# Priberam/Enhance-CB-Whisper

Hardware: AMD Instinct MI355X
Metric: utterances/sec (30 s clips) + keywords/sec matched, Whisper-large-v3 LEF 10k kw (higher is better)
Workload: dtype bf16

## Files before the change

enhance-cb-whisper_amd/cbw/_lib.py:

```python
from __future__ import annotations

import ctypes
import os

import torch

_HERE = os.path.dirname(os.path.abspath(__file__))
LIB_PATH = os.environ.get("CBW_LIB", os.path.join(_HERE, "libcbw.so"))

c_int, c_int64, c_float, c_void_p, c_char_p = ctypes.c_int, ctypes.c_int64, ctypes.c_float, ctypes.c_void_p, ctypes.c_char_p


class KwsConfig(ctypes.Structure):
    _fields_ = [("n_layers", c_int), ("embedding_dim", c_int), ("variant", c_int), ("proj_units", c_int),
                ("resnet_depth", c_int)]


class EncoderConfig(ctypes.Structure):
    _fields_ = [("n_mel", c_int), ("d_model", c_int), ("n_layers", c_int), ("n_heads", c_int), ("ffn_dim", c_int)]


class DecoderConfig(ctypes.Structure):
    _fields_ = [("vocab", c_int), ("d_model", c_int), ("n_layers", c_int), ("n_heads", c_int), ("ffn_dim", c_int),
                ("max_len", c_int)]
# ... 73 lines not shown
    "cbw_decoder_prefill": (c_int, [c_void_p, c_void_p, c_int, c_int, c_int, c_void_p, c_int64, c_void_p, c_void_p]),
    "cbw_decoder_cross_kv_slot": (c_int, [c_void_p, c_void_p, c_int, c_int, c_void_p, c_int64, c_int, c_void_p]),
    "cbw_decoder_prefill_rows": (c_int, [c_void_p, c_void_p, c_int, c_int, c_int, c_int, c_int, c_int, c_void_p, c_int64,
                                         c_void_p, c_void_p]),
    "cbw_decoder_step_rows": (c_int, [c_void_p, c_void_p, c_void_p, c_int, c_int, c_void_p, c_int64, c_void_p, c_void_p]),
    "cbw_decoder_reorder": (c_int, [c_void_p, c_void_p, c_int, c_int, c_int, c_void_p, c_int64, c_void_p]),
    "cbw_decoder_cross_attn_probs": (c_int, [c_void_p, c_void_p, c_int, c_void_p, c_int, c_int, c_int, c_void_p,
                                             c_int64, c_void_p, c_void_p]),
    "cbw_dtw": (c_int, [c_void_p, c_int, c_int, c_void_p, c_void_p, c_void_p]),
    "cbw_logprob_topk": (c_int, [c_void_p, c_int, c_int, c_int, c_void_p, c_int64, c_int, c_void_p, c_void_p, c_void_p]),
    "cbw_timestamp_rules": (c_int, [c_void_p, c_int, c_int, c_int, c_void_p, c_void_p, c_int, c_int, c_int, c_int,
                                    c_void_p, c_void_p]),
    "cbw_kws_profile_read": (c_int, [c_void_p, ctypes.POINTER(ctypes.c_double), ctypes.POINTER(ctypes.c_double), ctypes.POINTER(c_int)]),
    "cbw_kws_profile_records": (c_int, [c_void_p, c_void_p, c_void_p, c_void_p, c_int]),
    "cbw_kws_profile_tiers": (c_int, [c_void_p, c_void_p, c_int]),
    "cbw_kws_profile_kernels": (c_int, [c_void_p, c_void_p, c_int]),
    "cbw_kws_calibrate_fp8": (c_int, [c_void_p, c_void_p, c_void_p, c_void_p, c_void_p, c_int, c_int, c_int, c_void_p,
                                      c_int, c_float, c_void_p, c_int64, c_void_p]),
    "cbw_kws_score_fp8": (c_int, [c_void_p, c_void_p, c_void_p, c_void_p, c_void_p, c_int, c_int, c_int, c_void_p,
                                  c_int, c_void_p, c_int64, c_void_p]),
    "cbw_kws_set_score_offset_fp8": (c_int, [c_void_p, c_void_p]),
    "cbw_kws_fp8_scales": (c_int, [c_void_p, c_void_p, c_int]),
    "cbw_conv2d_fp8": (c_int, [c_void_p] * 5 + [c_float, c_void_p, c_float] + [c_int] * 9 + [c_void_p]),
    "cbw_fp8_probe": (c_int, [c_int, c_void_p, c_void_p, c_void_p, c_void_p, c_int, c_void_p]),
    "cbw_conv2d_f32": (c_int, [c_void_p] * 5 + [c_int] * 12 + [c_void_p]),
    "cbw_sim_maps_f32": (c_int, [c_void_p, c_void_p, c_int, c_void_p, c_void_p] + [c_int] * 5 + [c_void_p, c_void_p, c_int,
                                 c_void_p, c_int, c_int, c_void_p, c_void_p]),
    "cbw_maxpool_f32": (c_int, [c_void_p, c_void_p, c_int, c_int, c_int, c_int, c_void_p]),
    "cbw_pool_fc_f32": (c_int, [c_void_p] * 4 + [c_int, c_int, c_void_p, c_int, c_int, c_void_p]),
    "cbw_split3_f32": (c_int, [c_void_p, c_void_p, c_int64, c_int, c_void_p]),
    "cbw_channel_sum_workspace_bytes": (c_int64, [c_int]),
    "cbw_channel_sum_f32": (c_int, [c_void_p, c_int64, c_int, c_void_p, c_int64, c_void_p]),
    "cbw_conv2d_x3": (c_int, [c_void_p] * 4 + [c_int, c_void_p, c_void_p] + [c_int] * 9 + [c_void_p]),
}

ERRORS = {-1: "CBW_ERR_INVALID", -2: "CBW_ERR_HIP", -3: "CBW_ERR_OOM", -4: "CBW_ERR_STATE", -5: "CBW_ERR_NOT_FOUND"}

_lib = None


class CbwError(RuntimeError):
    pass


def load() -> ctypes.CDLL:
    global _lib
    if _lib is None:
        if not os.path.exists(LIB_PATH):
            raise CbwError(f"libcbw.so not found at {LIB_PATH}; build it with `python -c 'import __graft_entry__ as g; "
                           f"g.build()'` (hipcc --offload-arch=gfx950)")
        lib = ctypes.CDLL(LIB_PATH)
        for name, (res, args) in SIGNATURES.items():
            fn = getattr(lib, name)
            fn.restype = res
            fn.argtypes = args
        _lib = lib
    return _lib


def check(rc: int, what: str) -> None:
    if rc != 0:
        msg = load().cbw_last_error()
        msg = msg.decode() if msg else ""
        err = ValueError if rc == -1 else CbwError
        raise err(f"{what} failed with {ERRORS.get(rc, rc)}: {msg}")

# ... 25 lines not shown
```

enhance-cb-whisper_amd/csrc/cbw_kernels.h:

```cpp
#pragma once
#include <hip/hip_runtime.h>
#include <stdint.h>

#include <initializer_list>
#include <string>

typedef __bf16 bf16;

enum {
    CBW_EPI_RELU = 1,
    CBW_EPI_GELU = 2,
    CBW_EPI_RES_F32 = 4,
    CBW_EPI_OUT_F32 = 8,
    CBW_EPI_RES_AFTER_ACT = 16,
    CBW_EPI_SPLIT3 = 32,
    CBW_EPI_RES_SPLIT = 64
};

struct ConvArgs {
    const void* x;
    const void* w;
    const float* bias;
    const void* res;
    void* y;
    const void* zero;
    int N, H, W, Cin, Ho, Wo, Cout, KH, KW;
    int sh, sw, ph, pw;
    int M;
    int res_ld, y_ld;
    int flags;
    const void* x2;
    int Cin2, H2, W2, s2;
    int ksplit;
    float* partial;
    float* y32;
    int x_ld, xfold;
};

hipError_t cbw_conv_igemm(const ConvArgs& a, hipStream_t st);
extern thread_local const char* cbw_last_conv_kernel;
extern thread_local int cbw_cs_grid_cus;
inline std::string kernel_name(const char* base, std::initializer_list<int> targs) {
    std::string s = std::string(base) + "<";
    bool first = true;
    for (int t : targs) {
        s += (first ? "" : ", ") + std::to_string(t);
        first = false;
    }
    return s + ">";
}
int cbw_conv_splitk_factor(const ConvArgs& a);
hipError_t cbw_conv_igemm_splitk(const ConvArgs& a, int ksplit, float* partial, hipStream_t st);
struct GemvArgs {
    const bf16* x;
    int ldx;
    const bf16* w;
    const float* bias;
    const void* res;
    int res_ld;
    void* y;
    int ldy;
    int M, N, K, flags;
    const float* xf;
    const float* ln_g;
    const float* ln_b;
    float ln_eps;
    bf16* kv_k;
    bf16* kv_v;
    int64_t kv_ld;
// ... 148 lines not shown
```

enhance-cb-whisper_amd/csrc/conv_igemm.hip:

```cpp
#include "cbw_common.h"
#include "cbw_kernels.h"

thread_local const char* cbw_last_conv_kernel = "";

namespace {

constexpr int BK = 64;
constexpr int EPI_LD = 68;
constexpr int EPI_BYTES = 4 * 64 * EPI_LD * 4;
template <int BM, int BN>
constexpr int lds_bytes() { return 2 * (BM + BN) * 128 > EPI_BYTES ? 2 * (BM + BN) * 128 : EPI_BYTES; }

CBW_DEV int swz(int r) { return (r >> 1) & 7; }

CBW_DEV void store_out8(const ConvArgs& a, int flags, int m, int col, const float (&v)[8]) {
    if (flags & CBW_EPI_SPLIT3) {
        bf16x8 hi, lo;
#pragma unroll
        for (int q = 0; q < 8; ++q) {
            hi[q] = f2bf(v[q]);
            lo[q] = f2bf(v[q] - bf2f(hi[q]));
        }
        bf16* yp = (bf16*)a.y + (int64_t)m * a.y_ld + col;
        *(bf16x8*)yp = hi;
// ... 232 lines not shown
#pragma unroll
            for (int q = 0; q < 8; ++q) v[q] = fmaxf(v[q], 0.f);
        } else if (flags & CBW_EPI_GELU) {
#pragma unroll
            for (int q = 0; q < 8; ++q) v[q] = gelu_erf(v[q]);
        }
        if (has_res && (flags & CBW_EPI_RES_AFTER_ACT))
#pragma unroll
            for (int q = 0; q < 8; ++q) v[q] += rv[q];
        store_out8(a, flags, m, col, v);
    }
}

template <int BM, int BN, int KH, int KW>
__global__ __launch_bounds__(256, 2) void conv_igemm_persist(ConvArgs a, int ntiles) {
    static_assert((BM / 64) * (BN / 64) == 4, "4 waves x 64x64 tiles");
    static_assert(KH * KW <= 32, "tap mask");
    constexpr int STAGE = (BM + BN) * 128;
    constexpr int WN = BN / 64;
    constexpr int AR = BM / 32;
    constexpr int BR = BN / 32;
    extern __shared__ __attribute__((aligned(16))) char smem[];

    const int tid = threadIdx.x, lane = tid & 63, wid = tid >> 6;
    const int wm = wid / WN, wn = wid % WN;
    float* E = (float*)(smem + 2 * STAGE) + wid * 8 * EPI_LD;
    const int nt_n = a.Cout / BN;
    const int cin2 = (KH * KW == 1 && a.x2 != nullptr) ? a.Cin2 : 0;
    const int Ktot = KH * KW * a.Cin + cin2;
    const int csteps = a.Cin / BK;
    const int nsteps = KH * KW * csteps + cin2 / BK;
    const int HoWo = a.Ho * a.Wo;
    const int xld = a.x_ld ? a.x_ld : a.Cin;
    const int G = gridDim.x;
    const int my_tiles = (ntiles - (int)blockIdx.x + G - 1) / G;
    const int total = my_tiles * nsteps;
    const int sub_r = lane >> 3, chunk = lane & 7;
    auto tile_of = [&](int ti) { return xcd_remap(ti * G + (int)blockIdx.x, ntiles); };

    int64_t a_base[AR];
    int64_t a_base2[(KH * KW == 1) ? AR : 1];
    int a_ih0[AR], a_iw0[AR];
    bool a_ok[AR];
    const bf16* wrow[BR];
    const bool dual = (KH * KW == 1) && a.x2 != nullptr;
    const int csteps1 = csteps;
    auto setup_issue_tile = [&](int ti) {
        const int tile = tile_of(ti);
        const int m0 = (tile / nt_n) * BM, n0 = (tile % nt_n) * BN;
#pragma unroll
        for (int j = 0; j < AR; ++j) {
            const int r = (wid * AR + j) * 8 + sub_r;
            const int m = m0 + r;
            a_ok[j] = m < a.M;
            const int mm = a_ok[j] ? m : 0;
            const int n = mm / HoWo, rem = mm - n * HoWo;
            const int oh = rem / a.Wo, ow = rem - oh * a.Wo;
            a_ih0[j] = oh * a.sh - a.ph;
            a_iw0[j] = ow * a.sw - a.pw;
            a_base[j] = (int64_t)n * a.H * a.W * xld;
            if constexpr (KH * KW == 1)
                if (dual) a_base2[j] = (((int64_t)n * a.H2 + oh * a.s2) * a.W2 + ow * a.s2) * a.Cin2;
        }
#pragma unroll
        for (int j = 0; j < BR; ++j) {
            const int r = (wid * BR + j) * 8 + sub_r;
            wrow[j] = (const bf16*)a.w + (int64_t)(n0 + r) * Ktot + ((chunk ^ swz(r)) * 8);
        }
    };
    auto issue_stage = [&](int s, int buf) {
        const int tap = s / csteps;
        const int c0 = fold_c((s - tap * csteps) * BK, a.xfold);
        const int kh = tap / KW, kw = tap - kh * KW;
        char* A = smem + buf * STAGE;
        char* B = A + BM * 128;
        const bool second = dual && s >= csteps1;
#pragma unroll
        for (int j = 0; j < AR; ++j) {
            const int rb = wid * AR + j;
            const int r = rb * 8 + sub_r;
            const void* src;
            const int ih = a_ih0[j] + kh, iw = a_iw0[j] + kw;
            bool ok = a_ok[j];
            if constexpr (KH * KW > 1) ok = ok && ih >= 0 && ih < a.H && iw >= 0 && iw < a.W;
            if (!ok)
                src = a.zero;
            else if constexpr (KH * KW == 1) {
                if (second)
                    src = (const bf16*)a.x2 + a_base2[j] + (s - csteps1) * BK + ((chunk ^ swz(r)) * 8);
                else
                    src = (const bf16*)a.x + a_base[j] + ((int64_t)ih * a.W + iw) * xld + c0 + ((chunk ^ swz(r)) * 8);
            } else
                src = (const bf16*)a.x + a_base[j] + ((int64_t)ih * a.W + iw) * xld + c0 + ((chunk ^ swz(r)) * 8);
            __builtin_amdgcn_global_load_lds(src, (void*)(A + rb * 1024), 16, 0, 0);
        }
#pragma unroll
        for (int j = 0; j < BR; ++j) {
            const int rb = wid * BR + j;
            __builtin_amdgcn_global_load_lds((const void*)(wrow[j] + (int64_t)s * BK), (void*)(B + rb * 1024), 16, 0, 0);
        }
    };

    const int ecg = lane & 7, erow = lane >> 3;
    const bool res_bf16 = a.res != nullptr && !(a.flags & (CBW_EPI_RES_F32 | CBW_EPI_RES_SPLIT));
    bf16x8 rpre[8];
    f32x4 bias0, bias1;
    auto prefetch_epi = [&](int tile) {
        const int m0 = (tile / nt_n) * BM, n0 = (tile % nt_n) * BN;
        const int ecol = n0 + wn * 64 + ecg * 8;
#pragma unroll
        for (int it = 0; it < 8; ++it) {
            const int m = m0 + wm * 64 + it * 8 + erow;
            if (res_bf16 && m < a.M)
                rpre[it] = *(const bf16x8*)((const bf16*)a.res + (int64_t)m * a.res_ld + ecol);
            else
                rpre[it] = bf16x8{};
        }
        bias0 = f32x4{0.f, 0.f, 0.f, 0.f};
        bias1 = f32x4{0.f, 0.f, 0.f, 0.f};
        if (a.bias) {
            bias0 = *(const f32x4*)(a.bias + ecol);
            bias1 = *(const f32x4*)(a.bias + ecol + 4);
// ... 298 lines not shown
CBW_DEV int p8_off(int r, int c) { return r * 128 + ((c ^ ((r >> 1) & 7)) << 4); }
template <int BN> struct P8Shape {
    static constexpr int BM = 65536 / BN;
    static constexpr int NA = BM / 128, NB = BN / 128;
    static constexpr int WCN = BN / 64;
    static constexpr int BUF = (BM + BN) * 128;
};
template <int N> CBW_DEV void vm_wait() {
    static_assert(N >= 0 && N <= 15, "vm_wait");
    asm volatile("s_waitcnt vmcnt(%0)" ::"n"(N) : "memory");
}

template <int KH, int KW, int BN = 256>
__global__ __launch_bounds__(512, 1) void conv_igemm_p8(ConvArgs a) {
    static_assert(KH * KW <= 32, "tap mask");
    using S = P8Shape<BN>;
    constexpr int BM = S::BM, NA = S::NA, NB = S::NB, WCN = S::WCN;
    extern __shared__ __attribute__((aligned(16))) char smem[];
    const int tid = threadIdx.x, lane = tid & 63, wid = tid >> 6;
    const int wr = (wid >> 2) * (4 / WCN) + (wid & 3) / WCN, wc = (wid & 3) % WCN;
    const int fr = lane & 15, fq = lane >> 4;
    const int nt_n = a.Cout / BN;
    const int nt_m = (a.M + BM - 1) / BM;
    const int bid = xcd_remap(blockIdx.x, nt_m * nt_n);
    const int tm = bid / nt_n, tn = bid % nt_n;
    const int m0 = tm * BM, n0 = tn * BN;
    const int cin2 = a.x2 ? a.Cin2 : 0;
    const int Ktot = KH * KW * a.Cin + cin2;
    const int csteps = a.Cin / P8_BK;
    const int nk1 = KH * KW * csteps;
    const int nk = nk1 + cin2 / P8_BK;
    const int HoWo = a.Ho * a.Wo;
    const int xld = a.x_ld ? a.x_ld : a.Cin;

    const int sub = lane >> 3, pch = lane & 7;
    const bf16* a_px[2][NA];
    const bf16* a2_px[2][NA];
    unsigned a_tm[2][NA];
    const bf16* wrow[2][NB];
#pragma unroll
    for (int h = 0; h < 2; ++h)
#pragma unroll
        for (int g = 0; g < NA; ++g) {
            const int r = g * 128 + h * 64 + wid * 8 + sub;
            const int m = m0 + r;
            const bool okm = m < a.M;
            const int mm = okm ? m : 0;
            const int n = mm / HoWo, rem = mm - n * HoWo;
            const int oh = rem / a.Wo, ow = rem - oh * a.Wo;
            const int ih0 = oh * a.sh - a.ph, iw0 = ow * a.sw - a.pw;
            a2_px[h][g] = a.x2 ? (const bf16*)a.x2 + (((int64_t)n * a.H2 + oh * a.s2) * a.W2 + ow * a.s2) * cin2 +
                                     ((pch ^ ((r >> 1) & 7)) * 8)
                               : nullptr;
            unsigned tmask = 0;
#pragma unroll
            for (int kh = 0; kh < KH; ++kh)
#pragma unroll
                for (int kw = 0; kw < KW; ++kw) {
                    const int ih = ih0 + kh, iw = iw0 + kw;
                    if (okm && ih >= 0 && ih < a.H && iw >= 0 && iw < a.W) tmask |= 1u << (kh * KW + kw);
                }
            a_tm[h][g] = tmask;
            a_px[h][g] = (const bf16*)a.x + (int64_t)n * a.H * a.W * xld + ((int64_t)ih0 * a.W + iw0) * xld +
                         ((pch ^ ((r >> 1) & 7)) * 8);
        }
#pragma unroll
    for (int h = 0; h < 2; ++h)
#pragma unroll
        for (int g = 0; g < NB; ++g) {
            const int rb = h * (BN / 2) + g * 64 + wid * 8 + sub;
            const int rs = (rb & ~31) | (((rb & 15) >> 2) << 3) | (((rb >> 4) & 1) << 2) | (rb & 3);
            wrow[h][g] = (const bf16*)a.w + (int64_t)(n0 + rs) * Ktot + ((pch ^ ((rb >> 1) & 7)) * 8);
        }
    int nx_cs = 0, nx_tap = 0, nx_kh = 0, nx_kw = 0;
    int nx_off = fold_c(0, a.xfold);
    auto advance = [&]() {
        if (++nx_cs == csteps) {
            nx_cs = 0;
            ++nx_tap;
            if (++nx_kw == KW) { nx_kw = 0; ++nx_kh; }
        }
        nx_off = (nx_kh * a.W + nx_kw) * xld + fold_c(nx_cs * P8_BK, a.xfold);
    };
    auto issue = [&](int kt, int which) {
        char* A = smem + (kt & 1) * S::BUF;
        if (which == 0 || which == 3) {
            const int h = which == 3;
            if (kt >= nk1) {
                const int c0 = (kt - nk1) * P8_BK;
#pragma unroll
                for (int g = 0; g < NA; ++g) {
                    const void* src = (a_tm[h][g] & 1u) ? (const void*)(a2_px[h][g] + c0) : a.zero;
                    __builtin_amdgcn_global_load_lds(src, (void*)(A + (g * 128 + h * 64 + wid * 8) * 128), 16, 0, 0);
                }
                return;
            }
            const int tap = nx_tap;
            const int toff = nx_off;
#pragma unroll
            for (int g = 0; g < NA; ++g) {
                const void* src = ((a_tm[h][g] >> tap) & 1u) ? (const void*)(a_px[h][g] + toff) : a.zero;
                __builtin_amdgcn_global_load_lds(src, (void*)(A + (g * 128 + h * 64 + wid * 8) * 128), 16, 0, 0);
            }
        } else {
            const int h = which - 1;
            char* B = A + BM * 128;
#pragma unroll
            for (int g = 0; g < NB; ++g)
                __builtin_amdgcn_global_load_lds((const void*)(wrow[h][g] + (int64_t)kt * P8_BK),
                                                 (void*)(B + (h * (BN / 2) + g * 64 + wid * 8) * 128), 16, 0, 0);
        }
    };

    f32x4 acc[8][4];
#pragma unroll
    for (int i = 0; i < 8; ++i)
#pragma unroll
        for (int j = 0; j < 4; ++j) acc[i][j] = f32x4{0.f, 0.f, 0.f, 0.f};
    bf16x8 av[4][2], bv[2][2];

#pragma unroll
    for (int w = 0; w < 4; ++w) issue(0, w);
// ... 162 lines not shown

template <int BM, int BN, int KH, int KW>
hipError_t launch_persist(const ConvArgs& a, hipStream_t st) {
    const int ntiles = ((a.M + BM - 1) / BM) * (a.Cout / BN);
    int G = 2 * num_cus();
    if (ntiles < G) G = ntiles;
    constexpr int lds = 2 * (BM + BN) * 128 + 4 * 8 * EPI_LD * 4;
    static const std::string nm = kernel_name("conv_igemm_persist", {BM, BN, KH, KW});
    cbw_last_conv_kernel = nm.c_str();
    hipLaunchKernelGGL((conv_igemm_persist<BM, BN, KH, KW>), dim3(G), dim3(256), lds, st, a, ntiles);
    return hipGetLastError();
}

template <int BM, int BN, int KH, int KW>
hipError_t launch_t(const ConvArgs& a, hipStream_t st) {
    const int nt = ((a.M + BM - 1) / BM) * (a.Cout / BN);
    constexpr int lds = lds_bytes<BM, BN>();
    static const std::string nm = kernel_name("conv_igemm_kernel", {BM, BN, KH, KW});
    cbw_last_conv_kernel = nm.c_str();
    hipLaunchKernelGGL((conv_igemm_kernel<BM, BN, KH, KW>), dim3(nt), dim3(256), lds, st, a);
    return hipGetLastError();
}

bool ring_wanted(const ConvArgs& a) {
    if (!cbw_conv_ring_supported(a)) return false;
    const int ktot = a.KH * a.KW * a.Cin + (a.x2 ? a.Cin2 : 0);
    return a.KH * a.KW == 1 && a.res == nullptr && ktot <= 768;
}

template <int KH, int KW>
hipError_t launch_k(const ConvArgs& a, hipStream_t st) {
    const int64_t xld = a.x_ld ? a.x_ld : a.Cin;
    if (((int64_t)(KH - 1) * a.W + (KW - 1)) * xld + a.Cin + (a.x2 ? a.Cin2 : 0) > INT32_MAX) return hipErrorInvalidValue;
    const bool tile_only = a.xfold || (a.x_ld && a.x_ld != a.Cin) || (a.flags & (CBW_EPI_SPLIT3 | CBW_EPI_RES_SPLIT));
    const bool p8_fit = p8_mode() == 1 && a.res == nullptr && a.Cout % P8_BN == 0 && a.Cin % P8_BK == 0 &&
                        a.xfold % P8_BK == 0 && KH * KW * a.Cin + (a.x2 ? a.Cin2 : 0) >= 512 &&
                        (a.x2 == nullptr || (KH * KW == 1 && a.Cin2 % P8_BK == 0 && !a.xfold && !a.x_ld)) &&
                        !(a.flags & (CBW_EPI_OUT_F32 | CBW_EPI_GELU | CBW_EPI_RES_SPLIT)) &&
                        ((a.M + P8_BM - 1) / P8_BM) * (a.Cout / P8_BN) >= num_cus();
    const int px2 = p8_x2();
    if (p8_fit && a.x2 && px2 >= 2) return launch_p8<KH, KW>(a, st);
    if (!tile_only && KH * KW == 1 && cbw_conv_stream_wanted(a)) return cbw_conv_stream(a, st);
    if (p8_fit && a.x2 && px2 >= 1) return launch_p8<KH, KW>(a, st);
    if (p8_tier_enabled() && (a.flags & (CBW_EPI_SPLIT3 | CBW_EPI_OUT_F32)) && a.xfold && a.x2 == nullptr &&
        p8_mode() == 1 && a.Cout % P8_BN == 0 && a.Cin % P8_BK == 0 && a.xfold % P8_BK == 0 &&
        !(a.flags & (CBW_EPI_GELU | CBW_EPI_RES_AFTER_ACT))) {
        const int ktot = KH * KW * a.Cin;
        const int tiles = ((a.M + P8_BM - 1) / P8_BM) * (a.Cout / P8_BN);
        if (ktot >= 512 && (tiles >= num_cus() || (ktot >= 4096 && 2 * tiles >= num_cus())))
            return launch_p8<KH, KW>(a, st);
    }
    if (!tile_only && ring_wanted(a)) return cbw_conv_ring(a, st);
    const bool big_ok = a.res == nullptr && a.x2 == nullptr &&
                        !(a.flags & (CBW_EPI_OUT_F32 | CBW_EPI_GELU | CBW_EPI_RES_SPLIT)) &&
                        a.Cin % BIG_BK == 0 && a.xfold % BIG_BK == 0 && KH * KW * a.Cin >= 256;
    const int big_tiles = ((a.M + BIG_BM - 1) / BIG_BM) * (a.Cout / 256);
    if (big_ok && big_tiles >= num_cus()) {
        if (a.Cout % 256 == 0 && p8_mode() == 1 && a.Cin % P8_BK == 0 && a.xfold % P8_BK == 0)
            return launch_p8<KH, KW>(a, st);
        if (a.Cout % 256 == 0) return launch_big<256, KH, KW>(a, st);
    }
    if (big_ok && p8_n128() && p8_mode() == 1 && a.Cout % 256 == 128 && a.Cin % P8_BK == 0 && a.xfold % P8_BK == 0 &&
        KH * KW * a.Cin >= 512 && ((a.M + 511) / 512) * (a.Cout / 128) >= num_cus())
        return launch_p8<KH, KW, 128>(a, st);
    if (a.Cout % 128 == 0) {
        const bool short_k = a.KH * a.KW * (a.Cin / BK) == 1;
        if (a.x2 != nullptr || short_k || a.res != nullptr)
            return launch_persist<128, 128, KH, KW>(a, st);
        return launch_t<128, 128, KH, KW>(a, st);
    }
    if (a.x2 != nullptr) return hipErrorInvalidValue;
    return launch_t<256, 64, KH, KW>(a, st);
}

}

namespace {
__global__ __launch_bounds__(256) void splitk_epilogue_kernel(ConvArgs a, int S) {
    const int64_t n4 = (int64_t)a.M * a.Cout / 4;
    for (int64_t e = blockIdx.x * (int64_t)blockDim.x + threadIdx.x; e < n4; e += (int64_t)gridDim.x * blockDim.x) {
        const int64_t i = e * 4;
        const int m = (int)(i / a.Cout), col = (int)(i - (int64_t)m * a.Cout);
// ... 33 lines not shown
    }
}
}

int cbw_conv_splitk_factor(const ConvArgs& a) {
    if (a.KH != 1 || a.KW != 1 || a.x2 != nullptr || a.Cout % 128 || a.Cin % BK) return 1;
    const int tiles = ((a.M + 127) / 128) * (a.Cout / 128);
    const int slots = 2 * num_cus();
    const int nsteps = a.Cin / BK;
    int S = 1;
    while (S < 8 && tiles * (S * 2) <= slots && nsteps / (S * 2) >= 4) S *= 2;
    return S;
}

hipError_t cbw_conv_igemm_splitk(const ConvArgs& a0, int ksplit, float* partial, hipStream_t st) {
    if (ksplit <= 1 || partial == nullptr) return cbw_conv_igemm(a0, st);
    if (a0.KH != 1 || a0.KW != 1 || a0.x2 != nullptr || a0.Cout % 128 || a0.Cin % BK || a0.Cout % 4 ||
        a0.y_ld % 4 || (a0.res && a0.res_ld % 4) || ksplit > a0.Cin / BK)
        return hipErrorInvalidValue;
    ConvArgs a = a0;
    a.ksplit = ksplit;
    a.partial = partial;
    const int nt = ((a.M + 127) / 128) * (a.Cout / 128);
    constexpr int lds = lds_bytes<128, 128>();
    cbw_last_conv_kernel = "conv_igemm_kernel<128, 128, 1, 1> + splitk_epilogue_kernel";
    hipLaunchKernelGGL((conv_igemm_kernel<128, 128, 1, 1>), dim3(nt, ksplit), dim3(256), lds, st, a);
    const int64_t n4 = (int64_t)a.M * a.Cout / 4;
    const int grid = (int)std::min<int64_t>((n4 + 255) / 256, 4 * num_cus());
    hipLaunchKernelGGL(splitk_epilogue_kernel, dim3(grid), dim3(256), 0, st, a, ksplit);
    return hipGetLastError();
}

hipError_t cbw_conv_igemm(const ConvArgs& a, hipStream_t st) {
    if (a.x2 != nullptr && (a.KH != 1 || a.KW != 1 || a.Cin2 % BK)) return hipErrorInvalidValue;
    if (a.KH == 1 && a.KW == 1) return launch_k<1, 1>(a, st);
    if (a.KH == 3 && a.KW == 3) return launch_k<3, 3>(a, st);
    if (a.KH == 1 && a.KW == 3) return launch_k<1, 3>(a, st);
    return hipErrorInvalidValue;
}
```

enhance-cb-whisper_amd/csrc/runtime.cpp:

```cpp
#include <hip/hip_runtime.h>

#include <algorithm>
#include <cmath>
#include <cstring>
#include <limits>
#include <map>
#include <memory>
#include <string>
#include <vector>

#include "cbw.h"
#include "cbw_kernels.h"

namespace {

thread_local std::string g_err;

int fail(int code, const std::string& msg) {
    g_err = msg;
    return code;
}

#define HIPCHK(expr)                                                                                   \
    do {                                                                                               \
// ... 318 lines not shown
struct BlockW {
    ConvW conv[3];
    int nconv = 0;
    bool has_sc = false;
    bool fused_sc = false;
    ConvW sc;
    DevBuf chain_w;
};

struct ConvF8 : ConvW {
    DevBuf alpha;
};
struct BlockF8 {
    ConvF8 conv[3];
    bool has_sc = false;
    ConvF8 sc;
    float s_x = 1.f, s_t1 = 1.f, s_t2 = 1.f, s_sc = 1.f;
    float s_out = 1.f;
    bool out_bf16 = false;
};

int load_conv_bn_x3(const ParamStore& ps, const std::string& prefix, const ConvShape& s, bool relu, ConvW& c) {
    std::vector<float> o, sh;
    CHK(fold_conv_host(ps, prefix, s.cin, s.cout, s.k, o, sh));
    const size_t taps = (size_t)s.cout * s.k * s.k;
    std::vector<uint16_t> w(taps * 3 * s.cin);
    for (size_t t = 0; t < taps; ++t) split3(&o[t * s.cin], s.cin, &w[t * 3 * s.cin]);
    static_cast<ConvShape&>(c) = {3 * s.cin, s.cout, s.k, s.stride, relu};
    CHK(c.w.upload(w));
    CHK(c.b.upload(sh));
    return CBW_OK;
}

int launch_conv_x3(const ConvShape& c, const void* w, const float* bias, const void* x, int N, int H, int W, void* y,
                   float* y32, const void* res, bool res_split, int flags, const void* zero, hipStream_t st, Prof* prof) {
    ConvArgs a{};
    a.x = x; a.w = w; a.bias = bias; a.res = res; a.y = y; a.y32 = y32; a.zero = zero;
    a.xfold = c.cin / 3; a.x_ld = 2 * (c.cin / 3);
    conv_geometry(a, c, N, H, W);
    a.res_ld = res_split ? 2 * c.cout : c.cout;
    a.y_ld = (flags & CBW_EPI_SPLIT3) ? 2 * c.cout : c.cout;
    a.flags = flags | (res ? (res_split ? CBW_EPI_RES_SPLIT : CBW_EPI_RES_F32) : 0) | (c.relu ? CBW_EPI_RELU : 0);
    int slot;
    CHK(Prof::begin(prof, st, &slot));
    cbw_last_conv_kernel = "?";
    HIPCHK(cbw_conv_igemm(a, st));
    return Prof::end(prof, slot, st, 2.0 * a.M * a.Cout * (double)a.Cin * a.KH * a.KW, cbw_last_conv_kernel, 1);
}
int launch_conv_x3(const ConvW& c, const void* x, int N, int H, int W, void* y, float* y32, const void* res,
                   bool res_split, int flags, const void* zero, hipStream_t st, Prof* prof) {
    return launch_conv_x3(c, c.w.p, c.b.as<float>(), x, N, H, W, y, y32, res, res_split, flags, zero, st, prof);
}

int launch_conv32(const ConvW& c, const float* x, int N, int H, int W, float* y, const float* res, bool relu,
                  hipStream_t st) {
    F32ConvArgs a{};
    a.x = x; a.w = c.w.as<float>(); a.bias = c.b.as<float>(); a.res = res; a.y = y;
    conv_geometry(a, c, N, H, W);
    a.relu = relu ? 1 : 0;
    HIPCHK(cbw_conv_f32(a, st));
    return CBW_OK;
}

bool sc_fusion_enabled() {
    const char* e = getenv("CBW_NO_SC_FUSION");
    return !(e && atoi(e) != 0);
}

constexpr int KWS_MAX_STREAMS = 4;
hipError_t side_stream_create(hipStream_t* s) {
    const char* e = getenv("CBW_KWS_PRIO");
    int prio = e ? atoi(e) : 0;
    int least = 0, greatest = 0;
    if (hipDeviceGetStreamPriorityRange(&least, &greatest) == hipSuccess)
        prio = std::max(greatest, std::min(least, prio));
    return hipStreamCreateWithPriority(s, hipStreamNonBlocking, prio);
}

int kws_streams() {
    const char* e = getenv("CBW_KWS_STREAMS");
    const int n = e ? atoi(e) : 3;
    return std::max(1, std::min(KWS_MAX_STREAMS, n));
}

int stem_channels(int n_layers) { return n_layers <= 4 ? 4 : 16; }

bool bottleneck_first_enabled() {
    const char* e = getenv("CBW_NO_BOTTLENECK_FIRST");
    return !(e && atoi(e));
}
bool fp8_q8_enabled() {
    const char* e = getenv("CBW_FP8_Q8");
    return !(e && atoi(e) == 0);
}
// ... 162 lines not shown
        CHK(h->tp_w.upload(tw));
        CHK(h->tp_b.upload(tb));
    }
    return CBW_OK;
}

int build_f32(cbw_kws* h) {
    const int L = h->cfg.n_layers;
    const std::string stem = "model.feature_extractor.embedder.embedder";
    CHK(load_conv_bn(h->ps, stem, stem_shape(L), h->stem32, true));
    if (3 * L <= 16) {
        std::vector<float> o, sh;
        CHK(fold_conv_host(h->ps, stem, L, 64, 7, o, sh));
        std::vector<uint16_t> w16((size_t)64 * 7 * 8 * 16, 0);
        for (int co = 0; co < 64; ++co)
            for (int kh = 0; kh < 7; ++kh)
                for (int kw = 0; kw < 7; ++kw)
                    split3(&o[(((size_t)co * 7 + kh) * 7 + kw) * L], L, &w16[(((size_t)co * 7 + kh) * 8 + kw) * 16]);
        CHK(h->stem16x3_w.upload(w16));
    }
    h->blocks32.clear();
    h->blocks3.clear();
    for (const BlockTopo& t : h->topo) {
        BlockW b, b3;
        b.nconv = b3.nconv = t.nconv;
        b.has_sc = b3.has_sc = t.has_sc;
        if (t.has_sc) {
            CHK(load_conv_bn(h->ps, t.prefix + ".shortcut", t.sc, b.sc, true));
            CHK(load_conv_bn_x3(h->ps, t.prefix + ".shortcut", t.sc, false, b3.sc));
        }
        for (int j = 0; j < t.nconv; ++j) {
            const std::string p = t.prefix + ".layer." + std::to_string(j);
            CHK(load_conv_bn(h->ps, p, t.conv[j], b.conv[j], true));
            CHK(load_conv_bn_x3(h->ps, p, t.conv[j], true, b3.conv[j]));
        }
        h->blocks32.push_back(std::move(b));
        h->blocks3.push_back(std::move(b3));
    }
    return CBW_OK;
}

uint8_t f2e4m3_host(float f) {
    const uint8_t sign = std::signbit(f) ? 0x80 : 0;
    float a = std::fabs(f);
    if (std::isnan(a)) return 0x7F;
    if (a >= 448.f) return sign | 0x7E;
    int e;
    const float fr = std::frexp(a, &e);
    if (a == 0.f) return sign;
    int E = e - 1;
    if (E < -6) {
        const float q = std::nearbyint(a * 512.f);
        return sign | (uint8_t)q;
    }
    float m = std::nearbyint((fr * 2.f - 1.f) * 8.f);
    if (m == 8.f) { m = 0.f; ++E; }
    if (E > 8 || (E == 8 && m == 7.f)) return sign | 0x7E;
    return sign | (uint8_t)(((E + 7) << 3) | (int)m);
}

float e4m3_value_host(uint8_t c) {
    const int e = (c >> 3) & 15, m = c & 7;
    const float v = e == 0 ? std::ldexp((float)m / 8.f, -6) : std::ldexp(1.f + (float)m / 8.f, e - 7);
    return (c & 0x80) ? -v : v;
}

int load_conv_f8(const ParamStore& ps, const std::string& prefix, const ConvShape& s, bool relu, float s_in, ConvF8& c,
// ... 1117 lines not shown
    float* maps = (float*)p; p += align_up(plan.maps * 4);
    float* stem = (float*)p; p += align_up(plan.stem * 4);
    float* X32 = (float*)p; p += align_up(plan.big * 4);
    float* SC32 = (float*)p; p += align_up(plan.big * 4);
    uint16_t* X3 = (uint16_t*)p; p += align_up(plan.big * 4);
    uint16_t* Y3 = (uint16_t*)p; p += align_up(plan.big * 4);
    uint16_t* T1 = (uint16_t*)p; p += align_up(plan.small * 4);
    uint16_t* T2 = (uint16_t*)p;
    const void* zp = h->zero.p;
    const size_t nb = h->blocks3.size();
    const int X3_CHUNK = x3_chunk();
    for (int c0 = 0; c0 < n_sel; c0 += X3_CHUNK) {
        const int cn = std::min(X3_CHUNK, n_sel - c0);
        CHK(sim_f32_pass(h, utt, utt_mask, kwd, kwd_mask, K, pr, sel, c0, cn, maps, Tk, Tu, st));
        const int Hs = out_dim(Tk, 7, 2), Ws = out_dim(Tu, 7, 2);
        int H = out_dim(Hs, 3, 2), W = out_dim(Ws, 3, 2), C = 64;
        if (h->stem16x3_w.p && !x3_stem32()) {
            uint16_t* m16 = (uint16_t*)stem;
            HIPCHK(cbw_maps_split16(maps, m16, cn, L, Tk, Tu, st));
            HIPCHK(cbw_stem16_pool_x3(m16, h->stem16x3_w.as<uint16_t>(), h->stem32.b.as<float>(), X3, cn, Tk, Tu, Hs,
                                      Ws, H, W, st));
        } else {
            CHK(launch_conv32(h->stem32, maps, cn, Tk, Tu, stem, nullptr, true, st));
            HIPCHK(cbw_maxpool_f32(stem, X32, cn, Hs, Ws, 64, H, W, st));
            HIPCHK(cbw_split3(X32, X3, (int64_t)cn * H * W, 64, st));
        }
        uint16_t *x3 = X3, *y3 = Y3;
        for (size_t bi = 0; bi < nb; ++bi) {
            const auto& b = h->blocks3[bi];
            const BlockDims d = block_dims(h->topo[bi], H, W);
            const int Ho = d.Ho, Wo = d.Wo;
            const void* res = x3;
            bool res_split = true;
            if (b.has_sc) {
                CHK(launch_conv_x3(b.sc, x3, cn, H, W, SC32, nullptr, nullptr, false, CBW_EPI_OUT_F32, zp, st,
                                   &h->prof));
                res = SC32;
                res_split = false;
            }
            float* out32 = bi + 1 == nb ? X32 : nullptr;
            if (b.nconv == 3) {
                CHK(launch_conv_x3(b.conv[0], x3, cn, H, W, T1, nullptr, nullptr, false, CBW_EPI_SPLIT3, zp, st,
                                   &h->prof));
                CHK(launch_conv_x3(b.conv[1], T1, cn, d.h1, d.w1, T2, nullptr, nullptr, false, CBW_EPI_SPLIT3, zp, st,
                                   &h->prof));
                CHK(launch_conv_x3(b.conv[2], T2, cn, Ho, Wo, y3, out32, res, res_split, CBW_EPI_SPLIT3, zp, st,
                                   &h->prof));
            } else {
                CHK(launch_conv_x3(b.conv[0], x3, cn, H, W, T1, nullptr, nullptr, false, CBW_EPI_SPLIT3, zp, st,
                                   &h->prof));
                CHK(launch_conv_x3(b.conv[1], T1, cn, Ho, Wo, y3, out32, res, res_split, CBW_EPI_SPLIT3, zp, st,
                                   &h->prof));
            }
            std::swap(x3, y3);
            H = Ho;
            W = Wo;
            C = b.conv[b.nconv - 1].cout;
        }
        HIPCHK(cbw_pool_fc_f32(X32, h->fc_w.as<float>(), h->fc_b.as<float>(), sel, c0, cn, logits, H * W, C, st));
    }
    return CBW_OK;
}

int cbw_kws_rescore_x3(cbw_kws* h, const float* utt, const float* utt_mask, const float* kwd, const float* kwd_mask,
                       int K, int Tk, int Tu, const int32_t* sel, int n_sel, float* logits, void* ws, int64_t ws_bytes,
                       cbw_stream_t stream) {
    if (!h || !utt || !utt_mask || !kwd || !kwd_mask || !logits || (n_sel > 0 && !sel))
        return fail(CBW_ERR_INVALID, "null argument");
    return rescore_x3_impl(h, utt, utt_mask, kwd, kwd_mask, K, one_utterance(K), Tk, Tu, sel, n_sel, logits, ws, ws_bytes,
                           (hipStream_t)stream);
}

int cbw_kws_rescore_x3_pairs(cbw_kws* h, const float* utt, const float* utt_mask, int B, const float* kwd,
                             const float* kwd_mask, int K, int Tk, int Tu, const int32_t* pair_utt,
                             const int32_t* pair_kwd, int P, const int32_t* sel, int n_sel, float* logits, void* ws,
                             int64_t ws_bytes, cbw_stream_t stream) {
    if (!h) return fail(CBW_ERR_INVALID, "null handle");
    const RescorePairs pr{B, pair_utt, pair_kwd, P};
    CHK(check_rescore_pairs(pr, K, n_sel));
    if (n_sel > 0 && (!utt || !utt_mask || !kwd || !kwd_mask || !logits || !sel))
// ... 997 lines not shown
int cbw_split3_f32(const float* x, uint16_t* y, int64_t M, int C, cbw_stream_t stream) {
    if (!x || !y || M <= 0 || C <= 0 || C % 4 || (((uintptr_t)x | (uintptr_t)y) & 15))
        return fail(CBW_ERR_INVALID, "cbw_split3_f32: null or misaligned operand, or C % 4 != 0");
    HIPCHK(cbw_split3(x, y, M, C, (hipStream_t)stream));
    return CBW_OK;
}

int64_t cbw_channel_sum_workspace_bytes(int C) {
    if (C <= 0) return fail(CBW_ERR_INVALID, "cbw_channel_sum_workspace_bytes: bad argument");
    return (int64_t)cbw_channel_sum_groups() * C * (int64_t)sizeof(float);
}

int cbw_channel_sum_f32(const float* x, int64_t M, int C, float* part, int64_t part_bytes, cbw_stream_t stream) {
    if (!x || !part || M <= 0 || C <= 0) return fail(CBW_ERR_INVALID, "cbw_channel_sum_f32: bad argument");
    if (part_bytes < cbw_channel_sum_workspace_bytes(C)) return fail(CBW_ERR_OOM, "cbw_channel_sum_f32: part too small");
    HIPCHK(cbw_channel_sum_f32(x, M, C, part, (hipStream_t)stream));
    return CBW_OK;
}

int cbw_conv2d_x3(const uint16_t* x, const uint16_t* w, const float* bias, const void* res, int res_split, void* y,
                  float* y32, int out_split, int N, int H, int W, int C, int Cout, int k, int stride, int relu,
                  cbw_stream_t stream) {
    if (!x || !w || !bias || !y || N <= 0 || H <= 0 || W <= 0 || C <= 0 || C % 64 || Cout <= 0 || Cout % 64 ||
        (k != 1 && k != 3) || (stride != 1 && stride != 2) || (y32 && !out_split))
        return fail(CBW_ERR_INVALID, "cbw_conv2d_x3: null operand, C or Cout not a multiple of 64, k not 1 / 3, stride "
                                     "not 1 / 2, or y32 without the split output");
    const void* zp = nullptr;
    CHK(block_zero_page(&zp));
    const ConvShape c{3 * C, Cout, k, stride, relu != 0};
    return launch_conv_x3(c, w, bias, x, N, H, W, y, y32, res, res_split != 0,
                          out_split ? CBW_EPI_SPLIT3 : CBW_EPI_OUT_F32, zp, (hipStream_t)stream, nullptr);
}

}
```

include/cbw.h:

```cpp
#ifndef CBW_H
#define CBW_H
#include <stdint.h>

#ifdef __cplusplus
extern "C" {
#endif

#define CBW_OK 0
#define CBW_ERR_INVALID (-1)
#define CBW_ERR_HIP (-2)
#define CBW_ERR_OOM (-3)
#define CBW_ERR_STATE (-4)
#define CBW_ERR_NOT_FOUND (-5)

typedef void* cbw_stream_t;
typedef struct cbw_kws cbw_kws;
typedef struct cbw_encoder cbw_encoder;

int cbw_version(void);
const char* cbw_last_error(void);
const char* cbw_source_id(void);

typedef struct {
    int n_layers;
// ... 138 lines not shown
                    cbw_stream_t stream);

int cbw_conv2d(const uint16_t* x, const uint16_t* w, const float* bias, const void* res, void* y, int N, int H, int W,
               int Cin, int Cout, int KH, int KW, int sh, int sw, int ph, int pw, int flags, cbw_stream_t stream);
int cbw_conv1x1_chain(const uint16_t* x, const uint16_t* we, const float* be, const uint16_t* res, const uint16_t* wr,
                      const float* br, uint16_t* y, uint16_t* t1, int N, int H, int W, cbw_stream_t stream);
int cbw_conv2d_fp8(const uint8_t* x, const uint8_t* w, const float* alpha, const float* bias, const uint8_t* res,
                   float res_scale, void* y, float y_scale, int out_bf16, int relu, int N, int H, int W, int Cin,
                   int Cout, int k, int stride, cbw_stream_t stream);
int cbw_fp8_probe(int what, const void* a, const void* b, void* out, void* out2, int n, cbw_stream_t stream);

int cbw_conv1x1_dual(const uint16_t* x, const uint16_t* x2, const uint16_t* w, const float* bias, const void* res,
                     void* y, int N, int H, int W, int Cin, int H2, int W2, int Cin2, int s2, int Cout, int flags,
                     cbw_stream_t stream);
int cbw_gemm_splitk_factor(int M, int K, int N);
int cbw_gemm(const uint16_t* x, const uint16_t* w, const float* bias, const void* res, void* y, int M, int K, int N,
             int flags, int ksplit, float* partial, int64_t partial_floats, cbw_stream_t stream);
int cbw_encoder_attention(const uint16_t* qkv, uint16_t* out, int B, int T, int H, cbw_stream_t stream);

int cbw_conv2d_f32(const float* x, const float* w, const float* bias, const float* res, float* y, int N, int H, int W,
                   int Cin, int Cout, int KH, int KW, int sh, int sw, int ph, int pw, int relu, cbw_stream_t stream);
int cbw_sim_maps_f32(const float* utt, const float* utt_mask, int B, const float* kwd, const float* kwd_mask, int K,
                     int L, int Tk, int Tu, int E, const int32_t* pair_utt, const int32_t* pair_kwd, int n_pairs,
                     const int32_t* sel, int p0, int P, float* out, cbw_stream_t stream);
int cbw_maxpool_f32(const float* x, float* y, int N, int H, int W, int C, cbw_stream_t stream);
int cbw_pool_fc_f32(const float* x, const float* w, const float* b, const int32_t* sel, int p0, int P, float* logits,
                    int HW, int C, cbw_stream_t stream);
int cbw_split3_f32(const float* x, uint16_t* y, int64_t M, int C, cbw_stream_t stream);
int64_t cbw_channel_sum_workspace_bytes(int C);
int cbw_channel_sum_f32(const float* x, int64_t M, int C, float* part, int64_t part_bytes, cbw_stream_t stream);
int cbw_conv2d_x3(const uint16_t* x, const uint16_t* w, const float* bias, const void* res, int res_split, void* y,
                  float* y32, int out_split, int N, int H, int W, int C, int Cout, int k, int stride, int relu,
                  cbw_stream_t stream);

#ifdef __cplusplus
}
#endif
#endif
```

Before: 6.199.

## Fuse projection shortcut into x3 bottleneck expand conv via dual-source K concatenation

For bottleneck blocks with a 1x1 projection shortcut in the split-bf16 (x3) path, the shortcut weights are concatenated onto the expand conv's K dimension and the biases summed at load time. The kernel reads a second folded, strided input through new x2_ld/x2fold fields. This drops the separate shortcut conv launch and its fp32 SC32 write and read-back. In exchange the fused GEMM has a longer K, and kernel dispatch (p8 tier, tile_only) changes for folded second sources. It is gated by an env var that defaults on.

```diff
diff --git a/enhance-cb-whisper_amd/cbw/_lib.py b/enhance-cb-whisper_amd/cbw/_lib.py
--- a/enhance-cb-whisper_amd/cbw/_lib.py
+++ b/enhance-cb-whisper_amd/cbw/_lib.py
@@ -129,6 +129,7 @@
     "cbw_channel_sum_workspace_bytes": (c_int64, [c_int]),
     "cbw_channel_sum_f32": (c_int, [c_void_p, c_int64, c_int, c_void_p, c_int64, c_void_p]),
     "cbw_conv2d_x3": (c_int, [c_void_p] * 4 + [c_int, c_void_p, c_void_p] + [c_int] * 9 + [c_void_p]),
+    "cbw_conv2d_x3_dual": (c_int, [c_void_p] * 6 + [c_int] * 10 + [c_void_p]),
 }
 
 ERRORS = {-1: "CBW_ERR_INVALID", -2: "CBW_ERR_HIP", -3: "CBW_ERR_OOM", -4: "CBW_ERR_STATE", -5: "CBW_ERR_NOT_FOUND"}
diff --git a/enhance-cb-whisper_amd/csrc/cbw_kernels.h b/enhance-cb-whisper_amd/csrc/cbw_kernels.h
--- a/enhance-cb-whisper_amd/csrc/cbw_kernels.h
+++ b/enhance-cb-whisper_amd/csrc/cbw_kernels.h
@@ -35,6 +35,7 @@
     float* partial;
     float* y32;
     int x_ld, xfold;
+    int x2_ld, x2fold;
 };
 
 hipError_t cbw_conv_igemm(const ConvArgs& a, hipStream_t st);
diff --git a/enhance-cb-whisper_amd/csrc/conv_igemm.hip b/enhance-cb-whisper_amd/csrc/conv_igemm.hip
--- a/enhance-cb-whisper_amd/csrc/conv_igemm.hip
+++ b/enhance-cb-whisper_amd/csrc/conv_igemm.hip
@@ -288,6 +288,7 @@
     const int nsteps = KH * KW * csteps + cin2 / BK;
     const int HoWo = a.Ho * a.Wo;
     const int xld = a.x_ld ? a.x_ld : a.Cin;
+    const int x2ld = a.x2_ld ? a.x2_ld : a.Cin2;
     const int G = gridDim.x;
     const int my_tiles = (ntiles - (int)blockIdx.x + G - 1) / G;
     const int total = my_tiles * nsteps;
@@ -316,7 +317,7 @@
             a_iw0[j] = ow * a.sw - a.pw;
             a_base[j] = (int64_t)n * a.H * a.W * xld;
             if constexpr (KH * KW == 1)
-                if (dual) a_base2[j] = (((int64_t)n * a.H2 + oh * a.s2) * a.W2 + ow * a.s2) * a.Cin2;
+                if (dual) a_base2[j] = (((int64_t)n * a.H2 + oh * a.s2) * a.W2 + ow * a.s2) * x2ld;
         }
 #pragma unroll
         for (int j = 0; j < BR; ++j) {
@@ -326,11 +327,11 @@
     };
     auto issue_stage = [&](int s, int buf) {
         const int tap = s / csteps;
-        const int c0 = fold_c((s - tap * csteps) * BK, a.xfold);
+        const bool second = dual && s >= csteps1;
+        const int c0 = second ? fold_c((s - csteps1) * BK, a.x2fold) : fold_c((s - tap * csteps) * BK, a.xfold);
         const int kh = tap / KW, kw = tap - kh * KW;
         char* A = smem + buf * STAGE;
         char* B = A + BM * 128;
-        const bool second = dual && s >= csteps1;
 #pragma unroll
         for (int j = 0; j < AR; ++j) {
             const int rb = wid * AR + j;
@@ -343,7 +344,7 @@
                 src = a.zero;
             else if constexpr (KH * KW == 1) {
                 if (second)
-                    src = (const bf16*)a.x2 + a_base2[j] + (s - csteps1) * BK + ((chunk ^ swz(r)) * 8);
+                    src = (const bf16*)a.x2 + a_base2[j] + c0 + ((chunk ^ swz(r)) * 8);
                 else
                     src = (const bf16*)a.x + a_base[j] + ((int64_t)ih * a.W + iw) * xld + c0 + ((chunk ^ swz(r)) * 8);
             } else
@@ -708,6 +709,7 @@
     const int nk = nk1 + cin2 / P8_BK;
     const int HoWo = a.Ho * a.Wo;
     const int xld = a.x_ld ? a.x_ld : a.Cin;
+    const int x2ld = a.x2_ld ? a.x2_ld : cin2;
 
     const int sub = lane >> 3, pch = lane & 7;
     const bf16* a_px[2][NA];
@@ -725,7 +727,7 @@
             const int n = mm / HoWo, rem = mm - n * HoWo;
             const int oh = rem / a.Wo, ow = rem - oh * a.Wo;
             const int ih0 = oh * a.sh - a.ph, iw0 = ow * a.sw - a.pw;
-            a2_px[h][g] = a.x2 ? (const bf16*)a.x2 + (((int64_t)n * a.H2 + oh * a.s2) * a.W2 + ow * a.s2) * cin2 +
+            a2_px[h][g] = a.x2 ? (const bf16*)a.x2 + (((int64_t)n * a.H2 + oh * a.s2) * a.W2 + ow * a.s2) * x2ld +
                                      ((pch ^ ((r >> 1) & 7)) * 8)
                                : nullptr;
             unsigned tmask = 0;
@@ -763,7 +765,7 @@
         if (which == 0 || which == 3) {
             const int h = which == 3;
             if (kt >= nk1) {
-                const int c0 = (kt - nk1) * P8_BK;
+                const int c0 = fold_c((kt - nk1) * P8_BK, a.x2fold);
 #pragma unroll
                 for (int g = 0; g < NA; ++g) {
                     const void* src = (a_tm[h][g] & 1u) ? (const void*)(a2_px[h][g] + c0) : a.zero;
@@ -992,22 +994,26 @@
 hipError_t launch_k(const ConvArgs& a, hipStream_t st) {
     const int64_t xld = a.x_ld ? a.x_ld : a.Cin;
     if (((int64_t)(KH - 1) * a.W + (KW - 1)) * xld + a.Cin + (a.x2 ? a.Cin2 : 0) > INT32_MAX) return hipErrorInvalidValue;
-    const bool tile_only = a.xfold || (a.x_ld && a.x_ld != a.Cin) || (a.flags & (CBW_EPI_SPLIT3 | CBW_EPI_RES_SPLIT));
+    const bool x2_folded = a.x2 && (a.x2fold || (a.x2_ld && a.x2_ld != a.Cin2));
+    const bool tile_only = a.xfold || (a.x_ld && a.x_ld != a.Cin) || x2_folded ||
+                           (a.flags & (CBW_EPI_SPLIT3 | CBW_EPI_RES_SPLIT));
     const bool p8_fit = p8_mode() == 1 && a.res == nullptr && a.Cout % P8_BN == 0 && a.Cin % P8_BK == 0 &&
                         a.xfold % P8_BK == 0 && KH * KW * a.Cin + (a.x2 ? a.Cin2 : 0) >= 512 &&
-                        (a.x2 == nullptr || (KH * KW == 1 && a.Cin2 % P8_BK == 0 && !a.xfold && !a.x_ld)) &&
+                        (a.x2 == nullptr ||
+                         (KH * KW == 1 && a.Cin2 % P8_BK == 0 && !a.xfold && !a.x_ld && !x2_folded)) &&
                         !(a.flags & (CBW_EPI_OUT_F32 | CBW_EPI_GELU | CBW_EPI_RES_SPLIT)) &&
                         ((a.M + P8_BM - 1) / P8_BM) * (a.Cout / P8_BN) >= num_cus();
     const int px2 = p8_x2();
     if (p8_fit && a.x2 && px2 >= 2) return launch_p8<KH, KW>(a, st);
     if (!tile_only && KH * KW == 1 && cbw_conv_stream_wanted(a)) return cbw_conv_stream(a, st);
     if (p8_fit && a.x2 && px2 >= 1) return launch_p8<KH, KW>(a, st);
-    if (p8_tier_enabled() && (a.flags & (CBW_EPI_SPLIT3 | CBW_EPI_OUT_F32)) && a.xfold && a.x2 == nullptr &&
+    if (p8_tier_enabled() && (a.flags & (CBW_EPI_SPLIT3 | CBW_EPI_OUT_F32)) && a.xfold &&
+        (a.x2 == nullptr || (KH * KW == 1 && a.Cin2 % P8_BK == 0 && a.x2fold % P8_BK == 0)) &&
         p8_mode() == 1 && a.Cout % P8_BN == 0 && a.Cin % P8_BK == 0 && a.xfold % P8_BK == 0 &&
         !(a.flags & (CBW_EPI_GELU | CBW_EPI_RES_AFTER_ACT))) {
-        const int ktot = KH * KW * a.Cin;
+        const int ktot = KH * KW * a.Cin + (a.x2 ? a.Cin2 : 0);
         const int tiles = ((a.M + P8_BM - 1) / P8_BM) * (a.Cout / P8_BN);
-        if (ktot >= 512 && (tiles >= num_cus() || (ktot >= 4096 && 2 * tiles >= num_cus())))
+        if (ktot >= 512 && (a.x2 || tiles >= num_cus() || (ktot >= 4096 && 2 * tiles >= num_cus())))
             return launch_p8<KH, KW>(a, st);
     }
     if (!tile_only && ring_wanted(a)) return cbw_conv_ring(a, st);
@@ -1107,7 +1113,7 @@
 }
 
 hipError_t cbw_conv_igemm(const ConvArgs& a, hipStream_t st) {
-    if (a.x2 != nullptr && (a.KH != 1 || a.KW != 1 || a.Cin2 % BK)) return hipErrorInvalidValue;
+    if (a.x2 != nullptr && (a.KH != 1 || a.KW != 1 || a.Cin2 % BK || a.x2fold % BK)) return hipErrorInvalidValue;
     if (a.KH == 1 && a.KW == 1) return launch_k<1, 1>(a, st);
     if (a.KH == 3 && a.KW == 3) return launch_k<3, 3>(a, st);
     if (a.KH == 1 && a.KW == 3) return launch_k<1, 3>(a, st);
diff --git a/enhance-cb-whisper_amd/csrc/runtime.cpp b/enhance-cb-whisper_amd/csrc/runtime.cpp
--- a/enhance-cb-whisper_amd/csrc/runtime.cpp
+++ b/enhance-cb-whisper_amd/csrc/runtime.cpp
@@ -374,11 +374,35 @@
     return CBW_OK;
 }
 
+int load_fused_expand_shortcut_x3(const ParamStore& ps, const std::string& expand, const std::string& shortcut, int mid,
+                                  int cin, int cout, ConvW& c) {
+    std::vector<float> we, be, ws, bs;
+    CHK(fold_conv_host(ps, expand, mid, cout, 1, we, be));
+    CHK(fold_conv_host(ps, shortcut, cin, cout, 1, ws, bs));
+    const size_t K = 3 * (size_t)(mid + cin);
+    std::vector<uint16_t> w((size_t)cout * K);
+    std::vector<float> b(cout);
+    for (int co = 0; co < cout; ++co) {
+        split3(&we[(size_t)co * mid], mid, &w[co * K]);
+        split3(&ws[(size_t)co * cin], cin, &w[co * K + 3 * (size_t)mid]);
+        b[co] = be[co] + bs[co];
+    }
+    static_cast<ConvShape&>(c) = {3 * mid, cout, 1, 1, true};
+    CHK(c.w.upload(w));
+    CHK(c.b.upload(b));
+    return CBW_OK;
+}
+
 int launch_conv_x3(const ConvShape& c, const void* w, const float* bias, const void* x, int N, int H, int W, void* y,
-                   float* y32, const void* res, bool res_split, int flags, const void* zero, hipStream_t st, Prof* prof) {
+                   float* y32, const void* res, bool res_split, int flags, const void* zero, hipStream_t st, Prof* prof,
+                   const Src2* src2 = nullptr) {
     ConvArgs a{};
     a.x = x; a.w = w; a.bias = bias; a.res = res; a.y = y; a.y32 = y32; a.zero = zero;
     a.xfold = c.cin / 3; a.x_ld = 2 * (c.cin / 3);
+    if (src2) {
+        a.x2 = src2->x; a.Cin2 = src2->cin; a.H2 = src2->H; a.W2 = src2->W; a.s2 = src2->stride;
+        a.x2fold = src2->cin / 3; a.x2_ld = 2 * (src2->cin / 3);
+    }
     conv_geometry(a, c, N, H, W);
     a.res_ld = res_split ? 2 * c.cout : c.cout;
     a.y_ld = (flags & CBW_EPI_SPLIT3) ? 2 * c.cout : c.cout;
@@ -387,11 +411,12 @@
     CHK(Prof::begin(prof, st, &slot));
     cbw_last_conv_kernel = "?";
     HIPCHK(cbw_conv_igemm(a, st));
-    return Prof::end(prof, slot, st, 2.0 * a.M * a.Cout * (double)a.Cin * a.KH * a.KW, cbw_last_conv_kernel, 1);
+    return Prof::end(prof, slot, st, 2.0 * a.M * a.Cout * ((double)a.Cin * a.KH * a.KW + (a.x2 ? a.Cin2 : 0)),
+                     cbw_last_conv_kernel, 1);
 }
 int launch_conv_x3(const ConvW& c, const void* x, int N, int H, int W, void* y, float* y32, const void* res,
-                   bool res_split, int flags, const void* zero, hipStream_t st, Prof* prof) {
-    return launch_conv_x3(c, c.w.p, c.b.as<float>(), x, N, H, W, y, y32, res, res_split, flags, zero, st, prof);
+                   bool res_split, int flags, const void* zero, hipStream_t st, Prof* prof, const Src2* src2 = nullptr) {
+    return launch_conv_x3(c, c.w.p, c.b.as<float>(), x, N, H, W, y, y32, res, res_split, flags, zero, st, prof, src2);
 }
 
 int launch_conv32(const ConvW& c, const float* x, int N, int H, int W, float* y, const float* res, bool relu,
@@ -402,6 +427,14 @@
     a.relu = relu ? 1 : 0;
     HIPCHK(cbw_conv_f32(a, st));
     return CBW_OK;
+}
+
+bool x3_fold_sc() {
+    static const bool on = [] {
+        const char* e = getenv("CBW_X3_FOLD_SC");
+        return !(e && atoi(e) == 0);
+    }();
+    return on;
 }
 
 bool sc_fusion_enabled() {
@@ -630,7 +663,13 @@
         for (int j = 0; j < t.nconv; ++j) {
             const std::string p = t.prefix + ".layer." + std::to_string(j);
             CHK(load_conv_bn(h->ps, p, t.conv[j], b.conv[j], true));
-            CHK(load_conv_bn_x3(h->ps, p, t.conv[j], true, b3.conv[j]));
+            if (t.nconv == 3 && j == 2 && t.has_sc && t.sc.k == 1 && t.conv[2].cout % 128 == 0 && x3_fold_sc()) {
+                CHK(load_fused_expand_shortcut_x3(h->ps, p, t.prefix + ".shortcut", t.conv[2].cin, t.sc.cin,
+                                                  t.conv[2].cout, b3.conv[2]));
+                b3.fused_sc = true;
+            } else {
+                CHK(load_conv_bn_x3(h->ps, p, t.conv[j], true, b3.conv[j]));
+            }
         }
         h->blocks32.push_back(std::move(b));
         h->blocks3.push_back(std::move(b3));
@@ -1814,7 +1853,10 @@
             const int Ho = d.Ho, Wo = d.Wo;
             const void* res = x3;
             bool res_split = true;
-            if (b.has_sc) {
+            const Src2 sc_src{x3, b.sc.cin, H, W, b.sc.stride};
+            if (b.has_sc && b.fused_sc) {
+                res = nullptr;
+            } else if (b.has_sc) {
                 CHK(launch_conv_x3(b.sc, x3, cn, H, W, SC32, nullptr, nullptr, false, CBW_EPI_OUT_F32, zp, st,
                                    &h->prof));
                 res = SC32;
@@ -1827,7 +1869,7 @@
                 CHK(launch_conv_x3(b.conv[1], T1, cn, d.h1, d.w1, T2, nullptr, nullptr, false, CBW_EPI_SPLIT3, zp, st,
                                    &h->prof));
                 CHK(launch_conv_x3(b.conv[2], T2, cn, Ho, Wo, y3, out32, res, res_split, CBW_EPI_SPLIT3, zp, st,
-                                   &h->prof));
+                                   &h->prof, b.fused_sc ? &sc_src : nullptr));
             } else {
                 CHK(launch_conv_x3(b.conv[0], x3, cn, H, W, T1, nullptr, nullptr, false, CBW_EPI_SPLIT3, zp, st,
                                    &h->prof));
@@ -2891,4 +2933,20 @@
                           out_split ? CBW_EPI_SPLIT3 : CBW_EPI_OUT_F32, zp, (hipStream_t)stream, nullptr);
 }
 
-}
+int cbw_conv2d_x3_dual(const uint16_t* x, const uint16_t* x2, const uint16_t* w, const float* bias, void* y, float* y32,
+                       int N, int H, int W, int C, int H2, int W2, int C2, int s2, int Cout, int relu,
+                       cbw_stream_t stream) {
+    if (!x || !x2 || !w || !bias || !y || N <= 0 || H <= 0 || W <= 0 || H2 <= 0 || W2 <= 0 || C <= 0 || C % 64 ||
+        C2 <= 0 || C2 % 64 || Cout <= 0 || Cout % 128 || (s2 != 1 && s2 != 2) || out_dim(H2, 1, s2) != H ||
+        out_dim(W2, 1, s2) != W)
+        return fail(CBW_ERR_INVALID, "cbw_conv2d_x3_dual: null operand, C or C2 not a multiple of 64, Cout not a "
+                                     "multiple of 128, s2 not 1 / 2, or H x W not x2's extent at stride s2");
+    const void* zp = nullptr;
+    CHK(block_zero_page(&zp));
+    const ConvShape c{3 * C, Cout, 1, 1, relu != 0};
+    const Src2 src2{x2, 3 * C2, H2, W2, s2};
+    return launch_conv_x3(c, w, bias, x, N, H, W, y, y32, nullptr, false, CBW_EPI_SPLIT3, zp, (hipStream_t)stream,
+                          nullptr, &src2);
+}
+
+}
diff --git a/include/cbw.h b/include/cbw.h
--- a/include/cbw.h
+++ b/include/cbw.h
@@ -194,6 +194,9 @@
 int cbw_conv2d_x3(const uint16_t* x, const uint16_t* w, const float* bias, const void* res, int res_split, void* y,
                   float* y32, int out_split, int N, int H, int W, int C, int Cout, int k, int stride, int relu,
                   cbw_stream_t stream);
+int cbw_conv2d_x3_dual(const uint16_t* x, const uint16_t* x2, const uint16_t* w, const float* bias, void* y, float* y32,
+                       int N, int H, int W, int C, int H2, int W2, int C2, int s2, int Cout, int relu,
+                       cbw_stream_t stream);
 
 #ifdef __cplusplus
 }
```

Result: no change. 6.242 (median of 6 runs) (+0.7%).
